# wcaarls/grl

Hardware: AMD Instinct MI355X
Metric: env-steps/sec (batched rollouts), pendulum SARSA-tc (higher is better)
Workload: dtype f64

## Files before the change

grl_amd/capi.py:

```python
import ctypes as C
import os

from . import _build

MAX_DIMS, MAX_STATE, MAX_ACTIONS = 8, 12, 8

OK, ERR_INVALID, ERR_NO_DEVICE, ERR_HIP, ERR_TABLE_FULL, ERR_DOMAIN, ERR_ROWS_FULL, ERR_OOM = 0, -1, -2, -3, -4, -5, -6, -7
ENV_PENDULUM, ENV_CART_POLE, ENV_ACROBOT, ENV_COMPASS_WALKER, ENV_CART_POLE_BALANCING, ENV_EXTERNAL = 0, 1, 2, 3, 4, 5
AGENT_SARSA, AGENT_Q, AGENT_AC, AGENT_EXPECTED_SARSA, AGENT_ADVANTAGE, AGENT_QV = 0, 1, 2, 3, 4, 5
TRACE_NONE, TRACE_REPLACING, TRACE_ACCUMULATING = 0, 1, 2
PARAM_ALPHA, PARAM_GAMMA, PARAM_LAMBDA, PARAM_EPSILON = 0, 1, 2, 3


class TileSpec(C.Structure):
    _fields_ = [("tilings", C.c_int32), ("memory", C.c_int32), ("dims", C.c_int32), ("safe", C.c_int32),
                ("resolution", C.c_double * MAX_DIMS), ("wrapping", C.c_double * MAX_DIMS)]


class LinearSpec(C.Structure):
    _fields_ = [("init_min", C.c_double), ("init_max", C.c_double), ("output_min", C.c_double),
                ("output_max", C.c_double), ("limit", C.c_int32), ("reserved", C.c_int32)]


class Config(C.Structure):
# ... 64 lines not shown
    "grlx_rows": (C.c_int, [C.c_void_p]),
    "grlx_read_rows": (C.c_int, [C.c_void_p, C.c_int, C.c_int, C.c_int, _P(C.c_int64), _P(C.c_int64), _P(C.c_double)]),
    "grlx_last_kernel": (C.c_int, [C.c_void_p]),
    "grlx_replicas_per_wave": (C.c_int, [C.c_void_p]),
    "grlx_read_row_times": (C.c_int, [C.c_void_p, C.c_int, C.c_int, C.c_int, _P(C.c_double)]),
    "grlx_curve_stats": (C.c_int, [C.c_void_p, C.c_int, C.c_int, C.c_void_p, C.c_void_p]),
    "grlx_curve_stats_grouped": (C.c_int, [C.c_void_p, C.c_int, C.c_int, C.c_int, C.c_void_p, C.c_void_p]),
    "grlx_set_replica_params": (C.c_int, [C.c_void_p, C.c_int, _P(C.c_double)]),
    "grlx_get_replica_params": (C.c_int, [C.c_void_p, C.c_int, _P(C.c_double)]),
    "grlx_step_counts": (C.c_int, [C.c_void_p, _P(C.c_uint64), _P(C.c_uint64)]),
    "grlx_get_env_state": (C.c_int, [C.c_void_p, C.c_int, _P(C.c_double)]),
    "grlx_get_rng": (C.c_int, [C.c_void_p, C.c_int, _P(C.c_uint64)]),
    "grlx_get_weights": (C.c_int, [C.c_void_p, C.c_int, C.c_int, _P(C.c_uint32), C.c_int, _P(C.c_double)]),
    "grlx_table_load": (C.c_int, [C.c_void_p, C.c_int, C.c_int, _P(C.c_uint32)]),
    "grlx_table_capacity": (C.c_int, [C.c_void_p, _P(C.c_uint32)]),
    "grlx_grow_tables": (C.c_int, [C.c_void_p, C.c_uint32]),
    "grlx_reset_run": (C.c_int, [C.c_void_p]),
    "grlx_run_steps": (C.c_int, [C.c_void_p, C.c_int, C.c_uint64, C.c_void_p]),
    "grlx_replica_rows": (C.c_int, [C.c_void_p, C.c_int]),
    "grlx_get_target_weights": (C.c_int, [C.c_void_p, C.c_int, _P(C.c_uint32), C.c_int, _P(C.c_double), _P(C.c_uint32)]),
    "grlx_export_weights": (C.c_int, [C.c_void_p, C.c_int, C.c_int, _P(C.c_double)]),
    "grlx_load_weights": (C.c_int, [C.c_void_p, C.c_int, C.c_int, C.c_int, _P(C.c_double), C.c_uint64]),
    "grlx_snapshot_size": (C.c_int, [C.c_void_p, _P(C.c_uint64)]),
    "grlx_snapshot_save": (C.c_int, [C.c_void_p, C.c_void_p, C.c_uint64, _P(C.c_uint64)]),
    "grlx_snapshot_load": (C.c_int, [C.c_void_p, C.c_void_p, C.c_uint64]),
    "grlx_snapshot_info": (C.c_int, [C.c_void_p, C.c_uint64, _P(SnapshotInfo)]),
    "grlx_read_taps": (C.c_int, [C.c_void_p, _P(Tap), C.c_int, _P(C.c_int)]),
    "grlx_env_start": (C.c_int, [C.c_void_p, C.c_int, _P(C.c_int32), _P(C.c_double)]),
    "grlx_env_advance": (C.c_int, [C.c_void_p, _P(C.c_int32), _P(C.c_double), _P(C.c_double), _P(C.c_double), _P(C.c_int32)]),
    "grlx_agent_start": (C.c_int, [C.c_void_p, C.c_int, _P(C.c_int32), _P(C.c_double), _P(C.c_double)]),
    "grlx_agent_step": (C.c_int, [C.c_void_p, C.c_int, _P(C.c_int32), C.c_double, _P(C.c_double), _P(C.c_double), _P(C.c_int32), _P(C.c_double)]),
    "grlx_agent_end": (C.c_int, [C.c_void_p, C.c_int, _P(C.c_int32), C.c_double, _P(C.c_double), _P(C.c_double)]),
    "grlx_project": (C.c_int, [_P(TileSpec), _P(C.c_double), C.c_int, _P(C.c_uint32)]),
    "grlx_env_step": (C.c_int, [_P(Config), _P(C.c_double), _P(C.c_double), C.c_int, _P(C.c_double), _P(C.c_double), _P(C.c_int32)]),
    "grlx_env_dims": (C.c_int, [C.c_int, _P(C.c_int), _P(C.c_int)]),
    "grlx_read": (C.c_int, [C.c_void_p, C.c_int, _P(C.c_int32), _P(C.c_uint32), C.c_int, _P(C.c_double)]),
    "grlx_write": (C.c_int, [C.c_void_p, C.c_int, _P(C.c_int32), _P(C.c_uint32), C.c_int, _P(C.c_double), C.c_double]),
    "grlx_update": (C.c_int, [C.c_void_p, C.c_int, _P(C.c_int32), _P(C.c_uint32), C.c_int, _P(C.c_double)]),
    "grlx_math": (C.c_int, [C.c_int, _P(C.c_double), _P(C.c_double), C.c_int, _P(C.c_double)]),
    "grlx_rand48_at": (C.c_int, [C.c_int64, _P(C.c_uint64), C.c_int, _P(C.c_double)]),
    "grlx_fqi_config_pendulum": (None, [_P(FqiConfig)]),
    "grlx_fqi_create": (C.c_int, [_P(FqiConfig), _P(C.c_int64), _P(C.c_void_p)]),
    "grlx_fqi_destroy": (C.c_int, [C.c_void_p]),
    "grlx_fqi_run_batch": (C.c_int, [C.c_void_p, C.c_void_p]),
    "grlx_fqi_sync": (C.c_int, [C.c_void_p, C.c_void_p]),
    "grlx_fqi_read_rows": (C.c_int, [C.c_void_p, C.c_int, C.c_int, C.c_int, _P(C.c_int64), _P(C.c_int64), _P(C.c_double)]),
    "grlx_fqi_get_params": (C.c_int, [C.c_void_p, C.c_int, _P(C.c_double), C.c_int]),
    "grlx_fqi_get_transitions": (C.c_int, [C.c_void_p, C.c_int, C.c_int, C.c_int, _P(C.c_double), _P(C.c_double), _P(C.c_double), _P(C.c_double)]),
    "grlx_fqi_info": (C.c_int, [C.c_void_p, C.c_int, _P(C.c_int64), _P(C.c_double), _P(C.c_int32), _P(C.c_double), _P(C.c_uint64)]),
}

_DIAG_SIGS = {
    "grlx_env_server_counts": (C.c_int, [C.c_void_p, _P(C.c_int), _P(C.c_int)]),
    "grlx_env_server_debug": (C.c_int, [C.c_void_p, C.c_void_p, C.c_size_t]),
    "grlx_fqi_debug_stamps": (C.c_int, [C.c_void_p, _P(C.c_ulonglong), C.c_int]),
    "grlx_last_kernel_name": (C.c_char_p, [C.c_void_p]),
    "grlx_kernel_plan": (C.c_int, [_P(Config), C.c_int, C.c_int, _P(C.c_int), _P(C.c_int), _P(C.c_int), C.c_char_p, C.c_char_p, C.c_size_t]),
    "grlx_snapshot_timing": (C.c_int, [C.c_void_p, _P(C.c_double), _P(C.c_double)]),
    "grlx_snapshot_naive_copy": (C.c_int, [C.c_void_p, _P(C.c_uint64), _P(C.c_double), _P(C.c_double)]),
}
_NEWER_SIGS = ("grlx_snapshot_size", "grlx_snapshot_save", "grlx_snapshot_load", "grlx_snapshot_info")
PLAN_STAMPS_IN_PLACE, PLAN_STAMPS_DEFERRED, PLAN_SWEEP, PLAN_SERVER_OFF, PLAN_WALKER_SERVER, PLAN_FITS_YES, PLAN_FITS_NO = 1, 2, 4, 8, 16, 32, 64
ABI_VERSION = 2


def lib_path() -> str:
    return os.environ.get("GRLX_LIB") or _build.LIB


def _share_hip_runtime_with_torch():
    import importlib.util
    try:
        spec = importlib.util.find_spec("torch")
    except (ImportError, ValueError):
        spec = None
    if spec is None or not spec.origin:
        return
    cand = os.path.join(os.path.dirname(spec.origin), "lib", "libamdhip64.so")
    if os.path.exists(cand):
        C.CDLL(cand, mode=C.RTLD_GLOBAL)


def load():
    global _lib
    if _lib is not None:
        return _lib
    path = lib_path()
    if not os.path.exists(path):
        raise ImportError(f"{path} is missing: build the HIP extension first (python -m grl_amd._build); "
                          "grl_amd has no CPU fallback")
    _share_hip_runtime_with_torch()
    lib = C.CDLL(path)
    for name, (res, args) in list(_SIGS.items()) + list(_DIAG_SIGS.items()):
        if (name in _DIAG_SIGS or name in _NEWER_SIGS) and os.environ.get("GRLX_LIB") and not hasattr(lib, name):
            continue
        fn = getattr(lib, name)
        fn.restype = res
        fn.argtypes = args
    if lib.grlx_abi_version() != ABI_VERSION:
        raise ImportError(f"libgrlx.so ABI version {lib.grlx_abi_version()}, this binding is written for {ABI_VERSION}: rebuild (python -m grl_amd._build)")
    tag = (lib.grlx_build_pipeline() or b"").decode()
    if tag != _build.PIPELINE:
        raise ImportError(f"{path} was not built by grl_amd._build (pipeline tag {tag!r}, expected {_build.PIPELINE!r}): a plain hipcc build skips the "
                          "exec-prologue filter and its kernels can read stale lanes (DESIGN.md 4.1f); run `python -m grl_amd._build`")
    _lib = lib
    return lib
# ... 14 lines not shown
```

grl_amd/csrc/grlx_api.cpp:

```cpp
#include <cfloat>
#include <cmath>
#include <cstdarg>
#include <cstdio>
#include <cstdlib>
#include <chrono>
#include <cstring>
#include <string>
#include <vector>
#include "grlx_internal.h"
#include "grlx_snapshot.h"
#include "../../include/grlx_diag.h"

using namespace grlx;

namespace {

thread_local std::string g_err;

int fail(int code, const char *fmt, ...)
{
  char buf[512];
  va_list ap;
  va_start(ap, fmt);
  vsnprintf(buf, sizeof(buf), fmt, ap);
// ... 868 lines not shown
    {
      facts.server = false;
      plan = plan_rollout(Pb, facts);
    }
    if (plan.server)
    {
      Pb.env_mail = ctx->env_mail;
      Pb.env_tune = 3u;
      if (const char *tune = getenv("GRLX_ENV_SERVER_TUNE")) Pb.env_tune = (uint32_t)strtoul(tune, nullptr, 0);
      HIP_TRY(hipMemsetAsync(ctx->env_mail, 0, (size_t)ctx->P.n_replicas * ctx->env_mail_bytes, (hipStream_t)stream));
      HIP_TRY(hipEventRecord(ctx->srv_go, (hipStream_t)stream));
      HIP_TRY(hipStreamWaitEvent(ctx->srv_stream, ctx->srv_go, 0));
    }
    HIP_TRY(launch_plan(plan, Pb, n, ctx->sweep_dev, (hipStream_t)stream, ctx->srv_stream));
    ctx->last_row = plan.row;
    if (plan.server)
    {
      HIP_TRY(hipEventRecord(ctx->srv_done, ctx->srv_stream));
      HIP_TRY(hipStreamWaitEvent((hipStream_t)stream, ctx->srv_done, 0));
    }
  }
  HIP_TRY(launch_max_load(ctx->P, ctx->n_tables, ctx->max_load, (hipStream_t)stream));
  ctx->trials_run += n_trials;
  return GRLX_OK;
}

int grlx_env_server_debug(grlx_ctx *ctx, void *out, size_t bytes)
{
  if (!ctx || !out) return fail(GRLX_ERR_INVALID, "bad argument");
  if (!ctx->env_mail) return fail(GRLX_ERR_INVALID, "the environment server has not run in this context");
  DRAIN(ctx);
  const size_t have = (size_t)ctx->P.n_replicas * ctx->env_mail_bytes;
  HIP_TRY(hipMemcpy(out, ctx->env_mail, bytes < have ? bytes : have, hipMemcpyDeviceToHost));
  return GRLX_OK;
}

int grlx_env_server_counts(grlx_ctx *ctx, int *served, int *fell_back)
{
  if (!ctx || !served || !fell_back) return fail(GRLX_ERR_INVALID, "bad argument");
  *served = *fell_back = 0;
  if (!ctx->env_mail) return GRLX_OK;
  DRAIN(ctx);
  std::vector<unsigned long long> flag((size_t)ctx->P.n_replicas);
  HIP_TRY(hipMemcpy2D(flag.data(), sizeof(unsigned long long), (const char *)ctx->env_mail + kEnvMailFlagOffset, ctx->env_mail_bytes,
                      sizeof(unsigned long long), (size_t)ctx->P.n_replicas, hipMemcpyDeviceToHost));
  for (unsigned long long f : flag)
  {
    if (f == 1u) ++*served;
    if (f == 2u) ++*fell_back;
  }
  return GRLX_OK;
}

int grlx_run(grlx_ctx *ctx, int n_trials, void *stream) { return run_trials(ctx, n_trials, 0, stream); }

int grlx_run_steps(grlx_ctx *ctx, int max_trials, uint64_t steps, void *stream)
{
  if (steps == 0) return fail(GRLX_ERR_INVALID, "grlx_run_steps: steps must be > 0 (grlx_run has no budget)");
  if (steps > (1ull << 40)) return fail(GRLX_ERR_INVALID, "grlx_run_steps: steps out of range");
  return run_trials(ctx, max_trials, steps, stream);
}

static int status_to_error(uint64_t st)
{
  if (st & ST_TABLE_FULL) return fail(GRLX_ERR_TABLE_FULL, "a replica's sparse weight table overflowed: raise table_log2_capacity");
  if (st & ST_TRACE_OVERFLOW) return fail(GRLX_ERR_INVALID, "register trace overflow");
  if (st & ST_BAD_POS) return fail(GRLX_ERR_INVALID, "internal error: a TD update was queued without a table position");
  if (st & ST_DOMAIN) return fail(GRLX_ERR_DOMAIN, "sin/cos argument outside |x| < 2^20");
  if (st & ST_ROWS_FULL) return fail(GRLX_ERR_ROWS_FULL, "more test rows than max_rows");
  return GRLX_OK;
}

int grlx_sync(grlx_ctx *ctx, void *stream)
{
  if (!ctx) return fail(GRLX_ERR_INVALID, "null ctx");
  uint64_t h[3];
  if ((hipStream_t)stream != ctx->run_stream) DRAIN(ctx);
  HIP_TRY(launch_step_counts(ctx->P, ctx->scratch, (hipStream_t)stream));
  HIP_TRY(hipMemcpyAsync(h, ctx->scratch, sizeof(h), hipMemcpyDeviceToHost, (hipStream_t)stream));
  HIP_TRY(hipStreamSynchronize((hipStream_t)stream));
  if ((hipStream_t)stream == ctx->run_stream) ctx->run_pending = false;
  return status_to_error(h[2]);
}

int grlx_step_counts(grlx_ctx *ctx, uint64_t *learn_steps, uint64_t *test_steps)
{
  if (!ctx) return fail(GRLX_ERR_INVALID, "null ctx");
  uint64_t h[3];
  DRAIN(ctx);
  HIP_TRY(launch_step_counts(ctx->P, ctx->scratch, nullptr));
  HIP_TRY(hipMemcpy(h, ctx->scratch, sizeof(h), hipMemcpyDeviceToHost));
  if (learn_steps) *learn_steps = h[0];
  if (test_steps) *test_steps = h[1];
  return GRLX_OK;
}

int grlx_rows(grlx_ctx *ctx)
{
  if (!ctx) return fail(GRLX_ERR_INVALID, "null ctx");
  ReplicaState s;
  DRAIN(ctx);
  if (hipMemcpy(&s, ctx->states, sizeof(s), hipMemcpyDeviceToHost) != hipSuccess) return fail(GRLX_ERR_HIP, "hipMemcpy failed");
  return (int)s.rows;
}

int grlx_replica_rows(grlx_ctx *ctx, int replica)
// ... 1075 lines not shown
```

grl_amd/csrc/grlx_env_server.h:

```cpp
#pragma once

namespace grlx {

struct __attribute__((aligned(16))) MailUnit { double v; unsigned long long seq; };
constexpr int kCandUnits = 5;
struct __attribute__((aligned(1024))) EnvMail {
  unsigned long long cmd[4];
  MailUnit reset[3];
  unsigned long long pad0[6];
  unsigned long long stats[16];
  MailUnit cand[2][3][kCandUnits];
  unsigned long long pad1[36];
};
static_assert(sizeof(EnvMail) == kEnvMailBytes, "one mailbox = kEnvMailBytes");
static_assert(offsetof(EnvMail, stats) + 15 * sizeof(unsigned long long) == kEnvMailFlagOffset, "the flag grlx_env_server_counts reads");

typedef __attribute__((address_space(1))) unsigned long long env_gu64;
typedef unsigned int mail_u32x4 __attribute__((ext_vector_type(4)));
#define GRLX_RLX_AGENT __ATOMIC_RELAXED, __HIP_MEMORY_SCOPE_AGENT
constexpr unsigned kMailReset = 3u, kMailExit = 4u;
constexpr unsigned kFetchPolls = 400u;
constexpr unsigned kFirstFetchPolls = 8000u;
constexpr unsigned kServerStartPolls = 20000u;
constexpr unsigned kServerIdlePolls = 400000u;

__device__ __forceinline__ void mail_store(void *p, unsigned long long v) { __hip_atomic_store((env_gu64 *)p, v, GRLX_RLX_AGENT); }
__device__ __forceinline__ unsigned long long mail_load(const void *p) { return __hip_atomic_load((env_gu64 *)p, GRLX_RLX_AGENT); }
__device__ __forceinline__ void mail_setprio(unsigned p)
{
  if (p == 1) __builtin_amdgcn_s_setprio(1);
  else if (p == 2) __builtin_amdgcn_s_setprio(2);
  else if (p == 3) __builtin_amdgcn_s_setprio(3);
}
__device__ __forceinline__ unsigned long long mail_clock()
{
  unsigned long long t;
  asm volatile("s_memtime %0\n\ts_waitcnt lgkmcnt(0)" : "=s"(t)::"memory");
  return t;
}

__device__ __forceinline__ void unit_store(MailUnit *p, double v, unsigned long long seq)
{
  const unsigned long long b = (unsigned long long)__double_as_longlong(v);
  mail_u32x4 d;
  d.x = (unsigned)b; d.y = (unsigned)(b >> 32); d.z = (unsigned)seq; d.w = (unsigned)(seq >> 32);
  asm volatile("global_store_dwordx4 %0, %1, off sc1\n\ts_nop 1" ::"v"(p), "v"(d) : "memory");
}
template <int I>
__device__ __forceinline__ void unit_store_at(MailUnit *p, double v, unsigned long long seq)
{
  const unsigned long long b = (unsigned long long)__double_as_longlong(v);
  mail_u32x4 d;
  d.x = (unsigned)b; d.y = (unsigned)(b >> 32); d.z = (unsigned)seq; d.w = (unsigned)(seq >> 32);
  asm volatile("global_store_dwordx4 %0, %1, off offset:%2 sc1\n\ts_nop 1" ::"v"(p), "v"(d), "n"(I * (int)sizeof(MailUnit)) : "memory");
}
template <int N>
__device__ __forceinline__ bool units_load(const MailUnit *p, unsigned long long seq, double *v)
{
  static_assert(N == 3, "");
  mail_u32x4 d[N];
  asm volatile("global_load_dwordx4 %0, %3, off sc1\n\t"
               "global_load_dwordx4 %1, %3, off offset:16 sc1\n\t"
               "global_load_dwordx4 %2, %3, off offset:32 sc1\n\t"
               "s_waitcnt vmcnt(0)"
               : "=&v"(d[0]), "=&v"(d[1]), "=&v"(d[2])
               : "v"(p)
               : "memory");
  bool ok = true;
#pragma unroll
  for (int i = 0; i < N; ++i)
  {
    ok = ok && (((unsigned long long)d[i].w << 32) | d[i].z) == seq;
    v[i] = __longlong_as_double((long long)(((unsigned long long)d[i].y << 32) | d[i].x));
  }
  return ok;
}

__device__ __forceinline__ void mail_send(EnvMail *m, unsigned long long seq, unsigned op) { mail_store(&m->cmd[seq & 3u], (seq << 8) | op); }
__device__ __forceinline__ void mail_send_reset(EnvMail *m, unsigned long long seq, const double *x)
{
  unit_store(&m->reset[0], x[0], seq);
  unit_store(&m->reset[1], x[1], seq);
  unit_store(&m->reset[2], x[2], seq);
  mail_send(m, seq, kMailReset);
}

struct MailBox {
  __amdgpu_buffer_rsrc_t rs;
  unsigned at;
};
__device__ __forceinline__ MailBox mailbox_of(const DevParams &P, int r, int j)
{
  MailBox b;
  b.rs = __builtin_amdgcn_make_buffer_rsrc((void *)P.env_mail, 0, (int)((size_t)P.n_replicas * kEnvMailBytes), 0x00020000);
  b.at = (unsigned)r * (unsigned)kEnvMailBytes + (unsigned)offsetof(EnvMail, cand) + (unsigned)(j < kCandUnits ? j : 0) * (unsigned)sizeof(MailUnit);
  return b;
}
__device__ __forceinline__ mail_u32x4 mail_prefetch(const MailBox &b, unsigned long long seq, int a)
{
  const unsigned off = b.at + (((unsigned)seq & 1u) * 3u + (unsigned)a) * (unsigned)(kCandUnits * sizeof(MailUnit));
  return __builtin_amdgcn_raw_buffer_load_b128(b.rs, off, 0, 16);
}
template <int ENV>
__device__ __forceinline__ bool mail_take(const DevParams &N, const MailBox &b, mail_u32x4 d, unsigned long long seq, int a, int g,
                                          unsigned long long gmask, double *x, double *obs, double &reward, int &terminal, uint32_t &status,
                                          unsigned long long *polled = nullptr)
{
  static_assert(ENV == GRLX_ENV_PENDULUM, "the pendulum's mailbox");
  bool ok = false;
  unsigned polls = 0;
  for (;;)
  {
    const bool mine = (((unsigned long long)d.w << 32) | d.z) == seq;
    if ((__ballot(mine) & gmask) == gmask) { ok = true; break; }
    if (++polls > (seq <= 1u ? kFirstFetchPolls : kFetchPolls)) break;
    d = mail_prefetch(b, seq, a);
  }
  if (polled) *polled += polls;
  if (!ok) return false;
  const double v = __longlong_as_double((long long)(((unsigned long long)d.y << 32) | d.x));
  const int base = g * 16;
  x[0] = lane_fetch(v, base + 0);
  x[1] = lane_fetch(v, base + 1);
  x[2] = lane_fetch(v, base + 2);
  obs[0] = lane_fetch(v, base + 3);
  obs[1] = x[1];
  reward = lane_fetch(v, base + 4);
  terminal = x[2] > N.timeout ? 1 : 0;
  if (!Env<ENV>::in_domain(x)) status |= ST_DOMAIN;
  return true;
}

template <int ENV, int NA, typename SPEC>
__global__ __launch_bounds__(64) __attribute__((amdgpu_num_vgpr(48))) void env_server_kernel(DevParams P)
{
  static_assert(NA == 3, "sixteen lanes per replica: nine pairs of actions");
  constexpr int S = Env<ENV>::S, D = Env<ENV>::D;
  static_assert(S == 3 && D == 2, "the pendulum's mailbox");
  const DevParams &N = SPEC::numeric(P);
  const int lane = threadIdx.x & 63;
  const int q = lane >> 4, c = lane & 15;
  const int a = c / NA, a2 = c % NA;
  const bool worker = c < NA * NA;
  const int r = blockIdx.x * kReplicasPerWave + q;
  bool done = r >= P.n_replicas || (P.env_tune & 64u) != 0;
  EnvMail *m = P.env_mail + (done ? 0 : r);
  const double act = N.actions[a2];
  unsigned long long expect = 1;
  double cx[S], cobs0 = 0, creward = 0;
#pragma unroll
  for (int i = 0; i < S; ++i) cx[i] = 0;
  unsigned idle = 0;
  bool seen = false;
  mail_setprio((P.env_tune >> 2) & 3u);
  const typename Env<ENV>::ServerConsts ec = Env<ENV>::server_consts();
#ifdef GRLX_ENV_SERVER_STATS
  unsigned long long t_begin = mail_clock(), t_busy = 0, n_cmd = 0, n_idle = 0, n_split = 0, n_batch = 0;
#endif
  const unsigned long long quit_after = (P.env_tune >> 8) & 0xFFFFu;
  for (;;)
  {
    if (quit_after != 0u && expect > quit_after) done = true;
    if (__all(done)) break;
    unsigned long long word = 0;
    bool ready = false;
    if (!done)
    {
      word = mail_load(&m->cmd[expect & 3u]);
      ready = (word >> 8) == expect;
      if ((word >> 8) > expect) done = true;
    }
    if (!__any(ready))
// ... 95 lines not shown
```

grl_amd/csrc/grlx_internal.h:

```cpp
#pragma once
#include <hip/hip_runtime.h>
#include <stdint.h>
#include "../../include/grlx.h"

namespace grlx {

constexpr int kLanesPerReplica = 16;
constexpr size_t kEnvMailBytes = 1024;
constexpr size_t kEnvMailFlagOffset = 128 + 15 * 8;
constexpr size_t kWideMailBytes = 2048;
constexpr size_t kAcParkBytes = 12 * 64 * 16 + 3 * 64 * 4;
constexpr int kReplicasPerWave = 4;
constexpr int kMaxTrace = 10;
constexpr int kMaxActions = GRLX_MAX_ACTIONS;
constexpr uint32_t kInvalidPos = 0xFFFFFFFFu;
constexpr int kMaxProbe = 2048;
constexpr int kAcOwnedMax = 64;

enum : uint32_t { ST_TABLE_FULL = 1u, ST_DOMAIN = 2u, ST_ROWS_FULL = 4u, ST_TRACE_OVERFLOW = 8u,
                  ST_BAD_POS = 16u };

struct __attribute__((aligned(16))) Entry {
  uint32_t key;
  uint32_t aux;
  double   val;
};

struct __attribute__((aligned(16))) ReplicaState {
  double   x[GRLX_MAX_STATE];
  uint64_t G;
  uint64_t TL;
  uint64_t S1, S2;
  uint64_t TL0;
  double   eps_decay;
  double   ac_decay, ac_noise;
  int64_t  tt, ss;
  uint64_t test_steps;
  uint32_t n_slots[2];
  uint32_t status;
  uint32_t rows;
  int32_t  tr_len;
  int32_t  pad0;
  double   tr_total;
  const double *lazy_base[2];
  int64_t  sync_count;
  uint32_t syncs;
  uint32_t syncs_base;
  const double *target_base;
};

struct __attribute__((aligned(16))) AgentRep {
  double  time;
  double  action;
  int32_t action_index;
  int32_t pad;
};

struct __attribute__((aligned(32))) SweepParams {
  double alpha, gamma, gl, epsilon;
};

struct TileParams {
// ... 139 lines not shown
```

grl_amd/csrc/grlx_rollout.h:

```cpp
#pragma once

namespace grlx {

__device__ __forceinline__ unsigned long long stamp()
{
  unsigned long long t;
  __builtin_amdgcn_sched_barrier(0);
  asm volatile("s_memtime %0\n\ts_waitcnt lgkmcnt(0)" : "=s"(t)::"memory");
  __builtin_amdgcn_sched_barrier(0);
  return t;
}
#ifdef GRLX_ENV_SERVER_STATS
#define GRLX_STAMPED (DIAG || SERVED)
#else
#define GRLX_STAMPED DIAG
#endif
#define DIAG_STAMP(slot)                                   \
  if (GRLX_STAMPED)                                        \
  {                                                        \
    unsigned long long now__ = stamp();                    \
    diag_sum[slot] += now__ - diag_last;                   \
    diag_last = now__;                                     \
  }

// ... 185 lines not shown
  __shared__ uint32_t sh_ms[4 * NA * 16];
  __shared__ uint32_t sh_mail[4];
  __shared__ double   sh_res[4 * 16];
  __shared__ uint64_t sh_jump[2048];
  jump_table_to_lds(sh_jump);

  const int lane = threadIdx.x & 63;
  const int g = lane >> 4, j = lane & 15;
  const int r_raw = blockIdx.x * kReplicasPerWave + g;
  const bool live = r_raw < P.n_replicas;
  const int r = live ? r_raw : 0;
  const bool tapped = live && (r == P.tap_replica);
  const unsigned long long gmask = 0xFFFFull << (16 * g);

  ReplicaState &RS = P.states[r];
  double x[S];
#pragma unroll
  for (int i = 0; i < S; ++i) x[i] = RS.x[i];
  uint64_t G = RS.G, TL = RS.TL, S1 = RS.S1;
  double eps_decay = RS.eps_decay;
  int64_t tt = RS.tt, ss = RS.ss;
  uint64_t test_steps = RS.test_steps;
  uint32_t status = RS.status, rows = RS.rows, inserted = 0;

  const typename SPEC::Rep rep = SPEC::replica(sweep, r);
  const Table tab = table_of(P, 0, r);
  ReplicaState RSc;
  RSc.TL0 = RS.TL0;
  RSc.lazy_base[0] = RS.lazy_base[0];
  UpdateParams up;
  up.out_min = N.lin.out_min;
  up.out_max = N.lin.out_max;
  up.limit = N.lin.limit != 0;
  up.ee = SPEC::gl(N, rep);
  up.cut = (N.trace_kind == GRLX_TRACE_REPLACING) ? 0.01 : 0.0001;
  up.use_trace = N.trace_kind == GRLX_TRACE_REPLACING;
  up.dW = up.dT = 0;

  double acts[NA];
#pragma unroll
  for (int a = 0; a < NA; ++a) acts[a] = N.actions[a];
  uint32_t key_act[NA];
#pragma unroll
  for (int a = 0; a < NA; ++a)
    key_act[a] = in_reg(murmur_key(tile_coord<T>(N.tile, D, tile_quant(N.tile, D, N.actions[a]), j)));
  const uint32_t key_j = in_reg(murmur_key(j));

  LaneShare lshare;
  lshare.src[0] = g * 16; lshare.src[1] = g * 16 + 1; lshare.src[2] = g * 16 + 2;
  lshare.role3 = j % 3; lshare.role2 = j & 1;

  constexpr bool EXT = SERVED;
  static_assert(!SERVED || (DEFER && !DIAG && !TAP && !ADV && ENV == GRLX_ENV_PENDULUM && NA == 3), "what the environment server works for");
  EnvMail *mail = nullptr;
  unsigned long long mseq = 0;
  bool srv = false;
#ifdef GRLX_ENV_SERVER_STATS
  unsigned long long st_wait = 0, st_polls = 0, st_fetch = 0, st_begin = mail_clock();
#endif
  MailBox mbox;
  mail_u32x4 mpre = {0u, 0u, 0u, 0u};
  if constexpr (EXT)
  {
    srv = live && P.env_mail != nullptr;
    mail = P.env_mail + r;
    mbox = mailbox_of(P, r, j);
    mail_setprio(P.env_tune & 3u);
  }

  TraceRegs tr;
  trace_init(tr);
  int tr_len_ref = 0;
  bool pd = false, pd_sh = false;
  double pd_dW = 0, pd_dT = 0, pd_wp = 0;
  uint32_t pd_pos = kInvalidPos;
  unsigned long long diag_sum[8] = {0, 0, 0, 0, 0, 0, 0, 0}, diag_last = 0;
  if (GRLX_STAMPED) diag_last = stamp();

  for (int trial = 0; trial < n_trials; ++trial)
  {
    const bool act = live && !(P.steps_budget != 0u && (uint64_t)ss >= P.steps_budget);
    if (!__any(act)) break;
    const int ti = N.test_interval;
    const int test = (ti >= 0 && tt % (ti + 1) == ti) ? 1 : 0;
    double total_reward = 0, time = 0;
    const int subtrials = (test && P.test_trials > 1) ? P.test_trials : 1;
    for (int st = 0; st < P.test_trials; ++st)
    {
    const bool episode = act && st < subtrials;
    if (!__any(episode)) break;
    double obs[D], reward = 0;
    int terminal = 0;
    bool running = episode;

    if (episode)
    {
      Env<ENV>::start(N, test, TL, G, x);
      Env<ENV>::observe(N, x, obs);
      if constexpr (EXT)
        if (srv)
        {
          ++mseq;
          if (j == 0) mail_send_reset(mail, mseq, x);
        }
    }
    double action = 0;
    int    action_index = 0;
    uint32_t p_pos = kInvalidPos, p_slot = 0;
    bool   p_sh = false;
    double wp_seen = 0;
    uint32_t pos_prev[NA];
#pragma unroll
    for (int a = 0; a < NA; ++a) pos_prev[a] = 0u;
    if (!test) tr_len_ref = 0;
    bool first = true;

    for (;;)
    {
      if (!__any(running || pd)) break;
      uint32_t slot[NA];
      Lookup lk[NA];
      BucketRegs br[NA];
      double wp = 0;
      double wprev[NA];
#pragma unroll
      for (int a = 0; a < NA; ++a) wprev[a] = 0;
      bool has_next = false, update = false;
      if (running)
      {
        DIAG_STAMP(0)
        if (!first)
        {
          bool stepped = false;
          if constexpr (EXT)
            if (srv)
            {
#ifdef GRLX_ENV_SERVER_STATS
              const unsigned long long tf0 = mail_clock();
              stepped = mail_take<ENV>(N, mbox, mpre, mseq - 1, action_index, g, gmask, x, obs, reward, terminal, status, &st_polls);
              st_wait += mail_clock() - tf0;
              ++st_fetch;
#else
              stepped = mail_take<ENV>(N, mbox, mpre, mseq - 1, action_index, g, gmask, x, obs, reward, terminal, status);
#endif
              if (!stepped)
              {
                srv = false;
                ++mseq;
                if (j == 0) mail_send(mail, mseq, kMailExit);
              }
            }
          if (!stepped)
            env_step<ENV, true, LaneShare>(N, x, action, obs, reward, terminal, status, lshare);
          total_reward += reward;
          time += 1;
        }
        has_next = first || !Env<ENV>::kAbsorbing || terminal != 2;
        update = !first && !test;
        DIAG_STAMP(1)

        if (has_next)
        {
          uint32_t hpre = 449u ^ (uint32_t)(D + 2);
#pragma unroll
          for (int i = 0; i < D; ++i)
            hpre = murmur_mix(hpre, tile_coord<T>(N.tile, i, tile_quant(N.tile, i, obs[i]), j));
          const uint32_t hpm = hpre * 0x5bd1e995u;
#pragma unroll
          for (int a = 0; a < NA; ++a)
          {
            uint32_t h = hpm ^ key_act[a];
// ... 298 lines not shown
          p_sh = pick<bool, NA>(sh, a_next);
          wp_seen = pick<double, NA>(w, a_next);
          if (ADV)
          {
#pragma unroll
            for (int a = 0; a < NA; ++a) pos_prev[a] = pos[a];
          }
        }
        if (!first && terminal) running = false;
        first = false;
      }
      if (DEFER && ev.pos != kInvalidPos) value_store(tab, ev.pos, ev.val);
    }

    if (!test) trace_flush(tr, tab, true);
    }

    if (act && (ti >= 0 ? test : 1))
    {
      if (rows < (uint32_t)P.max_rows)
      {
        if (j == 0)
        {
          size_t at = (size_t)rows * (size_t)P.n_replicas + (size_t)r;
          P.row_reward[at] = total_reward / (double)subtrials;
          P.row_time[at] = time / (double)subtrials;
          P.row_steps[at] = ss;
          P.row_trial[at] = (ti >= 0) ? (tt + 1 - (tt + 1) / (ti + 1)) : tt;
        }
        rows++;
      }
      else
        status |= ST_ROWS_FULL;
    }
    tt += act ? 1 : 0;
  }

  if (DIAG && P.diag_out && lane == 0)
    for (int k = 0; k < 8; ++k) P.diag_out[(size_t)blockIdx.x * 8 + k] = diag_sum[k];

  if constexpr (EXT)
  {
#ifdef GRLX_ENV_SERVER_STATS
    if (live && j == 0 && P.env_mail)
    {
      mail->stats[4] = mail_clock() - st_begin;
      mail->stats[5] = st_wait;
      mail->stats[6] = st_fetch;
      mail->stats[7] = st_polls;
      mail->stats[8] = srv ? 1 : 0;
      for (int k = 0; k < 8; ++k) mail->pad1[k] = diag_sum[k];
    }
#endif
    if (live && j == 0 && P.env_mail) mail->stats[15] = srv ? 1u : 2u;
    if (srv)
    {
      ++mseq;
      if (j == 0) mail_send(mail, mseq, kMailExit);
    }
  }

  uint32_t ins = inserted;
#pragma unroll
  for (int off = 8; off > 0; off >>= 1) ins += __shfl_xor(ins, off, 16);
  if (live && j == 0)
  {
#pragma unroll
    for (int i = 0; i < S; ++i) RS.x[i] = x[i];
    RS.G = G;
    RS.TL = TL;
    RS.S1 = S1;
    RS.eps_decay = eps_decay;
    RS.tt = tt;
    RS.ss = ss;
    RS.test_steps = test_steps;
    RS.n_slots[0] += ins;
    RS.rows = rows;
  }
  uint32_t st = status;
#pragma unroll
  for (int off = 8; off > 0; off >>= 1) st |= __shfl_xor(st, off, 16);
  if (live && j == 0) RS.status = st;
}

template <int ENV, int NA, bool DIAG, typename SPEC, bool DEFER = !DIAG, bool ADV = false, bool TAP = !DEFER>
__global__ __launch_bounds__(64) GRLX_ROLLOUT_OCCUPANCY void rollout_kernel(DevParams P, int n_trials)
{
  rollout_body<ENV, NA, DIAG, SPEC, DEFER, ADV, TAP, false>(P, n_trials);
}

template <int ENV, int NA>
__global__ __launch_bounds__(64) GRLX_ROLLOUT_OCCUPANCY void rollout_sweep_kernel(DevParams P, int n_trials, const SweepParams *sweep)
{
  rollout_body<ENV, NA, false, SpecSweep, true, false, false, false>(P, n_trials, sweep);
}

template <int NA, typename SPEC>
__global__ __launch_bounds__(64) __attribute__((amdgpu_num_vgpr(208))) void rollout_served_kernel(DevParams P, int n_trials)
{
  rollout_body<GRLX_ENV_PENDULUM, NA, false, SPEC, true, false, false, true>(P, n_trials);
}


}
```

grl_amd/runner.py:

```python
import ctypes as C
import math

import numpy as np

from . import capi


def pendulum_sarsa_config(n_replicas=1, **overrides) -> capi.Config:
    lib = capi.load()
    cfg = capi.Config()
    lib.grlx_config_pendulum_sarsa(C.byref(cfg))
    cfg.n_replicas = n_replicas
    for k, v in overrides.items():
        setattr(cfg, k, v)
    return cfg


def cart_pole_ac_config(n_replicas=1, **overrides) -> capi.Config:
    lib = capi.load()
    cfg = capi.Config()
    lib.grlx_config_cart_pole_ac(C.byref(cfg))
    cfg.n_replicas = n_replicas
    for k, v in overrides.items():
        setattr(cfg, k, v)
# ... 132 lines not shown
            self._ctx = C.c_void_p()

    def __del__(self):
        try:
            self.close()
        except Exception:
            pass

    def run(self, n_trials: int, stream: int = 0):
        capi.check(self.lib.grlx_run(self._ctx, int(n_trials), C.c_void_p(stream)))

    def run_steps(self, max_trials: int, steps: int, stream: int = 0):
        capi.check(self.lib.grlx_run_steps(self._ctx, int(max_trials), int(steps), C.c_void_p(stream)))

    def sync(self, stream: int = 0):
        capi.check(self.lib.grlx_sync(self._ctx, C.c_void_p(stream)))

    def replica_rows(self, replica: int) -> int:
        return capi.check(self.lib.grlx_replica_rows(self._ctx, int(replica)))

    def set_diag(self, enable: bool = True):
        capi.check(self.lib.grlx_set_diag(self._ctx, int(enable)))

    def read_diag(self):
        waves = (self.cfg.n_replicas + 3) // 4
        out = np.zeros((waves, 8), np.uint64)
        n = C.c_int()
        capi.check(self.lib.grlx_read_diag(self._ctx, _ptr(out, C.c_uint64), waves, C.byref(n)))
        return out[: n.value]

    def n_rows(self) -> int:
        return capi.check(self.lib.grlx_rows(self._ctx))

    def rows(self, replica: int, first: int = 0, count: int = None):
        if count is None:
            count = self.replica_rows(replica) - first
        trial = np.zeros(count, np.int64)
        steps = np.zeros(count, np.int64)
        reward = np.zeros(count, np.float64)
        capi.check(self.lib.grlx_read_rows(self._ctx, replica, first, count, _ptr(trial, C.c_int64),
                                           _ptr(steps, C.c_int64), _ptr(reward, C.c_double)))
        return trial, steps, reward

    def last_kernel(self) -> int:
        return self.lib.grlx_last_kernel(self._ctx)

    def last_kernel_name(self) -> str:
        return self.lib.grlx_last_kernel_name(self._ctx).decode()

    def env_server_counts(self):
        a, b = C.c_int(0), C.c_int(0)
        capi.check(self.lib.grlx_env_server_counts(self._ctx, C.byref(a), C.byref(b)))
        return a.value, b.value

    def replicas_per_wave(self) -> int:
        return self.lib.grlx_replicas_per_wave(self._ctx)

    def row_times(self, replica: int, first: int = 0, count: int = None):
        if count is None:
            count = self.n_rows() - first
        out = np.zeros(count, np.float64)
        capi.check(self.lib.grlx_read_row_times(self._ctx, replica, first, count, _ptr(out, C.c_double)))
        return out

    def curve_stats(self, out_dev_ptr: int, first: int, count: int, stream: int = 0):
        capi.check(self.lib.grlx_curve_stats(self._ctx, first, count, C.c_void_p(out_dev_ptr), C.c_void_p(stream)))

    def curve_stats_grouped(self, out_dev_ptr: int, first: int, count: int, group_size: int, stream: int = 0):
        capi.check(self.lib.grlx_curve_stats_grouped(self._ctx, first, count, int(group_size), C.c_void_p(out_dev_ptr), C.c_void_p(stream)))

    def set_replica_params(self, alpha=None, gamma=None, lambda_=None, epsilon=None):
        given = {}
        for name, values in (("alpha", alpha), ("gamma", gamma), ("lambda_", lambda_), ("epsilon", epsilon)):
            if values is None:
                continue
            v = np.ascontiguousarray(values, dtype=np.float64)
            if v.shape != (self.cfg.n_replicas,):
                raise ValueError("need one value per replica")
            given[name] = v
        if not given:
            return
        before = self.replica_params()
        applied = []
        try:
            for name in ("alpha", "epsilon"):
                if name in given:
                    self._set_param(name, given[name])
                    applied.append(name)
            if "gamma" in given and "lambda_" in given:
                applied += ["gamma", "lambda_"]
                self._set_gamma_lambda(before["lambda_"], given["gamma"], given["lambda_"])
            else:
                for name in ("gamma", "lambda_"):
                    if name in given:
                        self._set_param(name, given[name])
        except capi.GrlxError:
            if "gamma" in applied:
                self._set_gamma_lambda(self.replica_params()["lambda_"], before["gamma"], before["lambda_"])
            for name in applied:
                if name in ("alpha", "epsilon"):
                    self._set_param(name, before[name])
            raise

    _PARAMS = {"alpha": capi.PARAM_ALPHA, "gamma": capi.PARAM_GAMMA, "lambda_": capi.PARAM_LAMBDA, "epsilon": capi.PARAM_EPSILON}

    def _set_param(self, name, v):
# ... 268 lines not shown
```

include/grlx_diag.h:

```cpp
#ifndef GRLX_DIAG_H_
#define GRLX_DIAG_H_

#include "grlx.h"

#ifdef __cplusplus
extern "C" {
#endif

int grlx_env_server_counts(grlx_ctx *ctx, int *served, int *fell_back);
int grlx_env_server_debug(grlx_ctx *ctx, void *out, size_t bytes);
int grlx_fqi_debug_stamps(grlx_fqi_ctx *ctx, unsigned long long *out, int count);

#define GRLX_PLAN_STAMPS_IN_PLACE 1
#define GRLX_PLAN_STAMPS_DEFERRED 2
#define GRLX_PLAN_SWEEP           4
#define GRLX_PLAN_SERVER_OFF      8
#define GRLX_PLAN_WALKER_SERVER  16
#define GRLX_PLAN_FITS_YES       32
#define GRLX_PLAN_FITS_NO        64
const char *grlx_last_kernel_name(grlx_ctx *ctx);
int grlx_kernel_plan(const grlx_config *cfg, int simds, int flags, int *replicas_per_wave, int *variant, int *grid, char *rollout_name,
                     char *server_name, size_t name_cap);


int grlx_snapshot_timing(grlx_ctx *ctx, double *pack_ms, double *unpack_ms);
int grlx_snapshot_naive_copy(grlx_ctx *ctx, uint64_t *bytes, double *out_ms, double *back_ms);

#ifdef __cplusplus
}
#endif
#endif
```

Measured before the change: 704.3 million.

## Add wave-uniform fast path for served pendulum SARSA steps

Adds a specialised inner loop for the common case where every replica in the wave is running, served, and past its first step. The loop waits on the mailbox with a wave-wide all-ready poll and then runs a straight-line lookup, TD update, action choice and send sequence, skipping the general loop's divergent branches. It also keeps the mailbox pointer as a base plus register index, and records a per-replica count of fast-path passes that a new diagnostic API reads back. The cost is a large duplicated code path that must match the general loop's semantics, and extra code size and register pressure.

```diff
diff --git a/grl_amd/capi.py b/grl_amd/capi.py
--- a/grl_amd/capi.py
+++ b/grl_amd/capi.py
@@ -140,6 +140,7 @@
 
 _DIAG_SIGS = {
     "grlx_env_server_counts": (C.c_int, [C.c_void_p, _P(C.c_int), _P(C.c_int)]),
+    "grlx_uniform_pass_counts": (C.c_int, [C.c_void_p, _P(C.c_ulonglong), C.c_int]),
     "grlx_env_server_debug": (C.c_int, [C.c_void_p, C.c_void_p, C.c_size_t]),
     "grlx_fqi_debug_stamps": (C.c_int, [C.c_void_p, _P(C.c_ulonglong), C.c_int]),
     "grlx_last_kernel_name": (C.c_char_p, [C.c_void_p]),
diff --git a/grl_amd/csrc/grlx_api.cpp b/grl_amd/csrc/grlx_api.cpp
--- a/grl_amd/csrc/grlx_api.cpp
+++ b/grl_amd/csrc/grlx_api.cpp
@@ -944,6 +944,18 @@
   return GRLX_OK;
 }
 
+int grlx_uniform_pass_counts(grlx_ctx *ctx, unsigned long long *out, int count)
+{
+  if (!ctx || !out || count < 0) return fail(GRLX_ERR_INVALID, "bad argument");
+  const int n = count < ctx->P.n_replicas ? count : ctx->P.n_replicas;
+  for (int i = 0; i < count; ++i) out[i] = 0;
+  if (!ctx->env_mail || n == 0) return GRLX_OK;
+  DRAIN(ctx);
+  HIP_TRY(hipMemcpy2D(out, sizeof(unsigned long long), (const char *)ctx->env_mail + kEnvMailUniformOffset, ctx->env_mail_bytes,
+                      sizeof(unsigned long long), (size_t)n, hipMemcpyDeviceToHost));
+  return GRLX_OK;
+}
+
 int grlx_run(grlx_ctx *ctx, int n_trials, void *stream) { return run_trials(ctx, n_trials, 0, stream); }
 
 int grlx_run_steps(grlx_ctx *ctx, int max_trials, uint64_t steps, void *stream)
diff --git a/grl_amd/csrc/grlx_env_server.h b/grl_amd/csrc/grlx_env_server.h
--- a/grl_amd/csrc/grlx_env_server.h
+++ b/grl_amd/csrc/grlx_env_server.h
@@ -14,6 +14,7 @@
 };
 static_assert(sizeof(EnvMail) == kEnvMailBytes, "one mailbox = kEnvMailBytes");
 static_assert(offsetof(EnvMail, stats) + 15 * sizeof(unsigned long long) == kEnvMailFlagOffset, "the flag grlx_env_server_counts reads");
+static_assert(offsetof(EnvMail, stats) + 14 * sizeof(unsigned long long) == kEnvMailUniformOffset, "the count grlx_uniform_pass_counts reads");
 
 typedef __attribute__((address_space(1))) unsigned long long env_gu64;
 typedef unsigned int mail_u32x4 __attribute__((ext_vector_type(4)));
@@ -76,14 +77,24 @@
   return ok;
 }
 
+struct MailRef {
+  EnvMail *all;
+  uint32_t r;
+  __device__ __forceinline__ EnvMail *get() const { return all + in_reg(r); }
+  __device__ __forceinline__ EnvMail *operator->() const { return get(); }
+};
 __device__ __forceinline__ void mail_send(EnvMail *m, unsigned long long seq, unsigned op) { mail_store(&m->cmd[seq & 3u], (seq << 8) | op); }
 __device__ __forceinline__ void mail_send_reset(EnvMail *m, unsigned long long seq, const double *x)
 {
-  unit_store(&m->reset[0], x[0], seq);
-  unit_store(&m->reset[1], x[1], seq);
-  unit_store(&m->reset[2], x[2], seq);
+  static_assert(offsetof(EnvMail, reset) == 2 * sizeof(MailUnit), "reset[i] is unit 2 + i of the mailbox");
+  MailUnit *u = reinterpret_cast<MailUnit *>(m);
+  unit_store_at<2>(u, x[0], seq);
+  unit_store_at<3>(u, x[1], seq);
+  unit_store_at<4>(u, x[2], seq);
   mail_send(m, seq, kMailReset);
 }
+__device__ __forceinline__ void mail_send(const MailRef &m, unsigned long long seq, unsigned op) { mail_send(m.get(), seq, op); }
+__device__ __forceinline__ void mail_send_reset(const MailRef &m, unsigned long long seq, const double *x) { mail_send_reset(m.get(), seq, x); }
 
 struct MailBox {
   __amdgpu_buffer_rsrc_t rs;
@@ -118,6 +129,35 @@
   }
   if (polled) *polled += polls;
   if (!ok) return false;
+  const double v = __longlong_as_double((long long)(((unsigned long long)d.y << 32) | d.x));
+  const int base = g * 16;
+  x[0] = lane_fetch(v, base + 0);
+  x[1] = lane_fetch(v, base + 1);
+  x[2] = lane_fetch(v, base + 2);
+  obs[0] = lane_fetch(v, base + 3);
+  obs[1] = x[1];
+  reward = lane_fetch(v, base + 4);
+  terminal = x[2] > N.timeout ? 1 : 0;
+  if (!Env<ENV>::in_domain(x)) status |= ST_DOMAIN;
+  return true;
+}
+template <int ENV>
+__device__ __forceinline__ bool mail_take_wave(const DevParams &N, const MailBox &b, mail_u32x4 d, unsigned long long seq, int a, int g,
+                                               double *x, double *obs, double &reward, int &terminal, uint32_t &status,
+                                               unsigned long long *polled = nullptr)
+{
+  static_assert(ENV == GRLX_ENV_PENDULUM, "the pendulum's mailbox");
+  unsigned polls = 0;
+  while (!__all((((unsigned long long)d.w << 32) | d.z) == seq))
+  {
+    if (++polls > kFetchPolls)
+    {
+      if (polled) *polled += polls;
+      return false;
+    }
+    d = mail_prefetch(b, seq, a);
+  }
+  if (polled) *polled += polls;
   const double v = __longlong_as_double((long long)(((unsigned long long)d.y << 32) | d.x));
   const int base = g * 16;
   x[0] = lane_fetch(v, base + 0);
diff --git a/grl_amd/csrc/grlx_internal.h b/grl_amd/csrc/grlx_internal.h
--- a/grl_amd/csrc/grlx_internal.h
+++ b/grl_amd/csrc/grlx_internal.h
@@ -8,6 +8,7 @@
 constexpr int kLanesPerReplica = 16;
 constexpr size_t kEnvMailBytes = 1024;
 constexpr size_t kEnvMailFlagOffset = 128 + 15 * 8;
+constexpr size_t kEnvMailUniformOffset = 128 + 14 * 8;
 constexpr size_t kWideMailBytes = 2048;
 constexpr size_t kAcParkBytes = 12 * 64 * 16 + 3 * 64 * 4;
 constexpr int kReplicasPerWave = 4;
diff --git a/grl_amd/csrc/grlx_rollout.h b/grl_amd/csrc/grlx_rollout.h
--- a/grl_amd/csrc/grlx_rollout.h
+++ b/grl_amd/csrc/grlx_rollout.h
@@ -261,9 +261,10 @@
 
   constexpr bool EXT = SERVED;
   static_assert(!SERVED || (DEFER && !DIAG && !TAP && !ADV && ENV == GRLX_ENV_PENDULUM && NA == 3), "what the environment server works for");
-  EnvMail *mail = nullptr;
+  MailRef mail = {nullptr, 0u};
   unsigned long long mseq = 0;
   bool srv = false;
+  unsigned n_uniform = 0;
 #ifdef GRLX_ENV_SERVER_STATS
   unsigned long long st_wait = 0, st_polls = 0, st_fetch = 0, st_begin = mail_clock();
 #endif
@@ -272,7 +273,7 @@
   if constexpr (EXT)
   {
     srv = live && P.env_mail != nullptr;
-    mail = P.env_mail + r;
+    mail = MailRef{P.env_mail, (uint32_t)r};
     mbox = mailbox_of(P, r, j);
     mail_setprio(P.env_tune & 3u);
   }
@@ -326,6 +327,183 @@
 
     for (;;)
     {
+      if constexpr (SERVED)
+      {
+        static_assert(!Env<ENV>::kAbsorbing, "has_next is taken as true");
+        if (__all(live && running && !first && srv && !test && pd) && !(P.env_tune & 16u))
+        {
+          do
+          {
+            DIAG_STAMP(0)
+#ifdef GRLX_ENV_SERVER_STATS
+            const unsigned long long tf0 = mail_clock();
+            const bool stepped = mail_take_wave<ENV>(N, mbox, mpre, mseq - 1, action_index, g, x, obs, reward, terminal, status, &st_polls);
+            st_wait += mail_clock() - tf0;
+            ++st_fetch;
+#else
+            const bool stepped = mail_take_wave<ENV>(N, mbox, mpre, mseq - 1, action_index, g, x, obs, reward, terminal, status);
+#endif
+            if (!stepped) break;
+            ++n_uniform;
+            total_reward += reward;
+            time += 1;
+            DIAG_STAMP(1)
+
+            uint32_t slot[NA];
+            Lookup lk[NA];
+            BucketRegs br[NA];
+            {
+              uint32_t hpre = 449u ^ (uint32_t)(D + 2);
+#pragma unroll
+              for (int i = 0; i < D; ++i)
+                hpre = murmur_mix(hpre, tile_coord<T>(N.tile, i, tile_quant(N.tile, i, obs[i]), j));
+              const uint32_t hpm = hpre * 0x5bd1e995u;
+#pragma unroll
+              for (int a = 0; a < NA; ++a)
+              {
+                uint32_t h = hpm ^ key_act[a];
+                h = murmur_absorb(h, key_j);
+                const uint32_t hm = murmur_final(h), mem = (uint32_t)N.tile.memory;
+                slot[a] = ((mem & (mem - 1u)) == 0u) ? (hm & (mem - 1u)) : (hm % mem);
+              }
+            }
+            DIAG_STAMP(2)
+            __builtin_amdgcn_fence(__ATOMIC_SEQ_CST, "workgroup");
+            DIAG_STAMP(6)
+            double wp = wp_seen;
+            table_issue<NA>(tab, slot, lk, br);
+
+            Evicted ev;
+            ev.n = 0u; ev.pos = kInvalidPos; ev.val = 0;
+            DIAG_STAMP(7)
+            sh_ppos[g * 16 + j] = pd_pos;
+            sh_fbflag[j * 4 + g] = 0u;
+            wave_sync();
+            up.dW = pd_dW;
+            up.dT = pd_dT;
+            td_update_lane<true, true>(tr, tab, up, pd_pos, pd_sh, pd_wp, g, j, sh_ppos, sh_fb, sh_fbflag, status, ev);
+            DIAG_STAMP(5)
+
+            double q[NA];
+            uint32_t pos[NA];
+            double w[NA];
+            bool sh[NA];
+#pragma unroll
+            for (int a = 0; a < NA; ++a) { q[a] = 0; pos[a] = kInvalidPos; w[a] = 0; sh[a] = false; }
+            bool shared_event = false;
+            table_get_finish<NA>(tab, N.lin, RSc, 0, slot, lk, br, pos, w, sh, g, j, gmask, sh_mb, sh_ms, sh_mail, sh_jump, status, inserted,
+                                 [&](uint32_t mp) {
+                                   if (ev.pos != kInvalidPos && ev.pos == mp) value_store(tab, mp, ev.val);
+                                   trace_share_event(tr, tab, mp);
+                                   if (p_pos == mp) p_sh = true;
+                                   shared_event = true;
+                                 });
+            DIAG_STAMP(7)
+            if (rarely(__any(shared_event))) wp = value_load(tab, p_pos);
+            {
+              bool risky = ev.n > 1u || p_sh;
+#pragma unroll
+              for (int a = 0; a < NA; ++a) risky = risky || sh[a];
+              if (rarely(__any(risky)))
+              {
+#pragma unroll
+                for (int a = 0; a < NA; ++a) w[a] = value_load(tab, pos[a]);
+                wp = value_load(tab, p_pos);
+              }
+              const bool held = ev.pos != kInvalidPos;
+#pragma unroll
+              for (int a = 0; a < NA; ++a) w[a] = (held && pos[a] == ev.pos) ? ev.val : w[a];
+              wp = (held && p_pos == ev.pos) ? ev.val : wp;
+            }
+#pragma unroll
+            for (int a = 0; a < NA; ++a)
+            {
+              w[a] = trace_forward(tr, pos[a], w[a]);
+              SHW(a, j, g) = w[a];
+            }
+            wp = trace_forward(tr, p_pos, wp);
+            SHW(NA, j, g) = wp;
+            DIAG_STAMP(3)
+            wave_sync();
+            {
+              const int row = (j < NROWS) ? j : 0;
+              double sum = 0;
+#pragma unroll
+              for (int k = 0; k < 16; ++k) sum += SHW(row, k, g);
+              sum /= 16;
+              sh_res[g * 16 + j] = sum;
+            }
+            wave_sync();
+#pragma unroll
+            for (int a = 0; a < NA; ++a) q[a] = clampd(sh_res[g * 16 + a], up.out_min, up.out_max);
+            const double qsa = clampd(sh_res[g * 16 + NA], up.out_min, up.out_max);
+
+            int a_next = 0;
+            int mai = 0, man = 1;
+            double best = 0;
+            findmax<NA>(q, mai, man, best);
+            S1 = lcg_next(S1);
+            const double rnd = lcg_double(S1);
+            if (rnd < eps_decay * SPEC::epsilon(N, rep))
+            {
+              G = lcg_next(G);
+              a_next = (int)(lcg_long(G) % (uint32_t)NA);
+            }
+            else
+              a_next = (man > 1) ? tie_break<NA>(q, best, man, G) : mai;
+            if (!terminal)
+            {
+              ++mseq;
+              if (j == 0) mail_send(mail, mseq, (unsigned)a_next);
+              mpre = mail_prefetch(mbox, mseq - 1, a_next);
+            }
+
+            DIAG_STAMP(4)
+            {
+              double target = reward;
+              if (SPEC::agent(P) == GRLX_AGENT_SARSA)
+                target += SPEC::gamma(N, rep) * pick<double, NA>(q, a_next);
+              else if (SPEC::agent(P) == GRLX_AGENT_EXPECTED_SARSA)
+              {
+                const double de = eps_decay * SPEC::epsilon(N, rep);
+                double v = 0;
+#pragma unroll
+                for (int kk = 0; kk < NA; ++kk)
+                {
+                  double d = (q[kk] == best) ? 1. / man : 0.;
+                  if (d == 1) d = 1 - de;
+                  d += de / NA;
+                  v += q[kk] * d;
+                }
+                target += SPEC::gamma(N, rep) * v;
+              }
+              else
+              {
+                double v = -__builtin_inf();
+#pragma unroll
+                for (int kk = 0; kk < NA; ++kk) v = fmax(v, q[kk]);
+                target += SPEC::gamma(N, rep) * v;
+              }
+              const double delta = target - qsa;
+              pd_dW = SPEC::alpha(N, rep) * (target - qsa);
+              pd_dT = SPEC::alpha(N, rep) * delta;
+              pd_pos = p_pos;
+              status |= (p_pos == kInvalidPos) ? ST_BAD_POS : 0u;
+              pd_sh = p_sh;
+              pd_wp = wp;
+            }
+            DIAG_STAMP(5)
+            ss++;
+            action_index = a_next;
+            p_pos = pick<uint32_t, NA>(pos, a_next);
+            p_sh = pick<bool, NA>(sh, a_next);
+            wp_seen = pick<double, NA>(w, a_next);
+            if (terminal) running = false;
+            if (ev.pos != kInvalidPos) value_store(tab, ev.pos, ev.val);
+          } while (__all(running));
+          action = pick<double, NA>(acts, action_index);
+        }
+      }
       if (!__any(running || pd)) break;
       uint32_t slot[NA];
       Lookup lk[NA];
@@ -730,7 +908,11 @@
       for (int k = 0; k < 8; ++k) mail->pad1[k] = diag_sum[k];
     }
 #endif
-    if (live && j == 0 && P.env_mail) mail->stats[15] = srv ? 1u : 2u;
+    if (live && j == 0 && P.env_mail)
+    {
+      mail->stats[14] = n_uniform;
+      mail->stats[15] = srv ? 1u : 2u;
+    }
     if (srv)
     {
       ++mseq;
diff --git a/grl_amd/runner.py b/grl_amd/runner.py
--- a/grl_amd/runner.py
+++ b/grl_amd/runner.py
@@ -208,6 +208,11 @@
         a, b = C.c_int(0), C.c_int(0)
         capi.check(self.lib.grlx_env_server_counts(self._ctx, C.byref(a), C.byref(b)))
         return a.value, b.value
+
+    def uniform_pass_counts(self):
+        out = np.zeros(self.cfg.n_replicas, dtype=np.uint64)
+        capi.check(self.lib.grlx_uniform_pass_counts(self._ctx, _ptr(out, C.c_ulonglong), out.size))
+        return out
 
     def replicas_per_wave(self) -> int:
         return self.lib.grlx_replicas_per_wave(self._ctx)
diff --git a/include/grlx_diag.h b/include/grlx_diag.h
--- a/include/grlx_diag.h
+++ b/include/grlx_diag.h
@@ -8,6 +8,7 @@
 #endif
 
 int grlx_env_server_counts(grlx_ctx *ctx, int *served, int *fell_back);
+int grlx_uniform_pass_counts(grlx_ctx *ctx, unsigned long long *out, int count);
 int grlx_env_server_debug(grlx_ctx *ctx, void *out, size_t bytes);
 int grlx_fqi_debug_stamps(grlx_fqi_ctx *ctx, unsigned long long *out, int count);
 
```

New measurement: 728.5 million, median of 6. 1.03x the previous value.
